# KRLabsOrg/verbatim-rag

Measured on AMD Instinct MI355X. Metric: query x chunk span-extractions/sec @512tok (ModernBERT-base extractor, chunks/s), higher is better.
Workload: dtype bf16

## Files before the change

### include/vrag_amd_debug.h

```cpp
#ifndef VRAG_AMD_DEBUG_H
#define VRAG_AMD_DEBUG_H

#include <stdint.h>

#ifdef __cplusplus
extern "C" {
#endif

int vrag_debug_gemm_ms(int32_t epi, int32_t M, int32_t N, int32_t K, int32_t iters, int32_t device, float* ms_out);
int vrag_debug_attn_ms(int32_t local, int32_t n_seqs, int32_t S, int32_t H, int32_t window, int32_t iters, int32_t device,
                       float* ms_out);
int vrag_debug_qkv_attn_ms(int32_t local, int32_t n_seqs, int32_t S, int32_t H, int32_t window, int32_t iters, int32_t flags,
                           int32_t device, float* ms_out);
typedef struct vrag_debug_attn_args {
  const uint16_t* q;
  const uint16_t* k;
  const uint16_t* vt;
  uint16_t* o;
  const int32_t* seq_row;
  const int32_t* seq_len;
  int32_t* blocks_out;
  int32_t rows, H, n_seqs;
  int32_t local, window, f16;
  int32_t blocks_cap;
  int32_t n_blocks;
  int32_t f16_saturated;
} vrag_debug_attn_args;
int vrag_debug_attn_run_ex(vrag_debug_attn_args* args, int32_t device);
int vrag_debug_attn_run(int32_t local, int32_t n_seqs, int32_t S, int32_t H, int32_t window, int32_t f16, const uint16_t* q,
                        const uint16_t* k, const uint16_t* vt, uint16_t* o, int32_t device);

typedef struct vrag_debug_gemm_args {
  const uint16_t* A;
  const uint16_t* W;
  const float* bias;
  const float* ln_s;
  const float* stats_in;
  const float* res_mu;
  const float* res_rstd;
  const float* res_g;
  const float* res_b;
  const float* rope_cos;
  const float* rope_sin;
  const int32_t* pos;
  const int32_t* tok_seq;
  const uint8_t* lo_in;
  float* out_f32;
  uint16_t* out_bf16;
  uint16_t* q;
  uint16_t* k;
  uint16_t* vt;
  float* ln_mu;
  float* ln_rstd;
  float* ln_shift;
  float* ln_shift_prev;
  uint16_t* resid_bf16;
  float* stats_part;
  uint8_t* lo_out;
  uint32_t* splade_rows;
  int32_t epi, M, N, K, f16, act_gelu;
  int32_t row0, rows;
  int32_t hidden, rope_rows, n_seqs;
  int32_t small_rows;
  float q_scale, fin_eps;
  int32_t config[7];
  int32_t f16_saturated;
} vrag_debug_gemm_args;
int vrag_debug_gemm_run(vrag_debug_gemm_args* args, int32_t device);

typedef struct vrag_debug_qkv_attn_args {
  const uint16_t* x;
  const uint16_t* w;
  const float* ln_s;
  const float* ln_mu;
  const float* ln_rstd;
  const float* rope_cos;
  const float* rope_sin;
  uint16_t* o;
  const int32_t* seq_row;
  const int32_t* seq_len;
  int32_t* groups_out;
  int32_t rows, H, nh, rope_rows, n_seqs;
  int32_t packer;
  int32_t local, window, f16;
  float q_scale;
  int32_t n_groups;
  int32_t f16_saturated;
} vrag_debug_qkv_attn_args;
int vrag_debug_qkv_attn_run(vrag_debug_qkv_attn_args* args, int32_t device);
int vrag_debug_pack_groups(const int32_t* seq_row, const int32_t* seq_len, int32_t n, int32_t packer, int32_t* out);

enum {
  VRAG_DEBUG_ROWS_EMBED_LN = 0,
  VRAG_DEBUG_ROWS_LAYERNORM = 1,
  VRAG_DEBUG_ROWS_RANGE_POOL = 2,
  VRAG_DEBUG_ROWS_LN_CLASSIFIER = 3,
  VRAG_DEBUG_ROWS_POOLER_CLASSIFIER = 4,
  VRAG_DEBUG_ROWS_SEQ_HEAD = 5
};
typedef struct vrag_debug_rows_args {
  float* h;
  const int32_t* ids;
  const float* E;
  const float* P;
  const int32_t* pos;
  const float* type_row;
  const int32_t* type_ids;
  const float* w;
  const float* bias;
  const int32_t* start;
  const int32_t* end;
  const int32_t* first_row;
  const int32_t* seq_row;
  const int32_t* seq_len;
  const float* Wp;
  const float* bp;
  const float* WdT;
  const float* bd;
  const float* wn;
  const float* bn;
  const float* Wc;
  const float* bc;
  float* out_f32;
  uint16_t* out16;
  uint16_t* out_lo;
  float* row_mean;
  float* pooled;
  int32_t op, H, rows;
  int32_t h_rows, out_rows;
  int32_t vocab, n_pos, n_types;
  int32_t num_labels;
  int32_t mode;
  int32_t gelu_first, split3;
  int32_t alias_f32;
  int32_t f16;
  int32_t no_sat;
  float eps;
  int32_t launch_status;
  int32_t f16_saturated;
} vrag_debug_rows_args;
int vrag_debug_rows_run(vrag_debug_rows_args* args, int32_t device);

enum {
  VRAG_DEBUG_GLUE_CVT_ROWS = 0,
  VRAG_DEBUG_GLUE_CVT_SPLIT3 = 1,
  VRAG_DEBUG_GLUE_LN_STATS_FINALIZE = 2,
  VRAG_DEBUG_GLUE_PACK_LAYOUT = 3,
  VRAG_DEBUG_GLUE_SPLADE_COMPACT = 4,
  VRAG_DEBUG_GLUE_PERMUTE_QKV_HEADS = 5
};
typedef struct vrag_debug_glue_args {
  const float* src;
  const float* col_scale;
  uint16_t* dst;
  uint16_t* dst_lo;
  float* row_sum;
  const float* part;
  float* mu;
  float* rstd;
  const float* shift_in;
  float* shift_out;
  float* shift_prev;
  const int32_t* packed;
  const int32_t* seq_row;
  const int32_t* seq_src;
  const int32_t* seq_len;
  int32_t* ids;
  int32_t* pos;
  int32_t* tok_seq;
  int32_t* counts;
// ... 166 lines not shown
```

### verbatim-rag_amd/_lib.py

```python
from __future__ import annotations

import ctypes as C
import os
import threading

_HERE = os.path.dirname(os.path.abspath(__file__))
_LOCK = threading.Lock()
_LIB = None

VRAG_OK = 0
ABI_VERSION = 6
PROF_CLASSES = (
    "embed", "layernorm", "gemm_qkv", "attn_global", "attn_local",
    "gemm_wo", "gemm_wi", "gemm_wo_mlp", "head", "qkv_attn_global", "qkv_attn_local",
)


class VragError(RuntimeError):

    def __init__(self, fn: str, status: int, message: str):
        super().__init__(f"{fn} failed (status {status}): {message}")
        self.status = status


# ... 135 lines not shown
                                      _LP, _LP, C.c_int64, _IP, _IP, _LP]),
    "vrag_split_sentences": (C.c_int, [C.c_void_p, _LP, C.c_int32, C.c_int32, _IP, _IP, _IP, C.c_int32]),
    "vrag_topk_fill_empty": (C.c_int, [C.c_void_p, C.c_void_p, C.c_int64, C.c_int32, C.c_void_p]),
    "vrag_sparse_index_create": (C.c_int, [C.c_int32, C.c_int64, _LP, _IP, _FP, C.c_int32, C.POINTER(_H)]),
    "vrag_sparse_index_destroy": (None, [_H]),
    "vrag_sparse_index_stats": (C.c_int, [_H, _LP, _LP, _LP]),
    "vrag_sparse_index_search": (C.c_int, [_H, _LP, _IP, _FP, C.c_int32, C.c_int32, _FP, _LP, C.c_void_p]),
    "vrag_sparse_index_search_filtered": (C.c_int, [_H, _LP, _IP, _FP, C.c_int32, C.c_int32, C.c_void_p, C.c_int64, _FP, _LP,
                                                    C.c_void_p]),
    "vrag_sparse_index_run_resident": (C.c_int, [_H, C.c_int32, C.c_int32, C.c_void_p]),
    "vrag_text_tokenize": (C.c_int, [C.c_void_p, _LP, C.c_int32, C.c_int32, C.c_int64, _IP, C.c_void_p, _LP]),
    "vrag_text_index_create": (C.c_int, [C.c_float, C.c_float, C.c_int32, C.POINTER(_H)]),
    "vrag_text_index_destroy": (None, [_H]),
    "vrag_text_index_add": (C.c_int, [_H, C.c_void_p, _LP, C.c_int32, C.c_int32]),
    "vrag_text_index_set_live": (C.c_int, [_H, C.c_void_p, C.c_int64]),
    "vrag_text_index_stats": (C.c_int, [_H, _LP, _LP, _LP, _LP, _LP]),
    "vrag_text_index_set_corpus_stats": (C.c_int, [_H, C.c_int64, C.c_int64]),
    "vrag_text_index_query_terms": (C.c_int, [_H, C.c_void_p, _LP, C.c_int32, C.c_int64, _LP, C.c_void_p, _IP, _LP, _LP]),
    "vrag_text_index_search": (C.c_int, [_H, _LP, C.c_void_p, _FP, C.c_int32, C.c_int32, C.c_void_p, C.c_int64, _FP, _LP]),
    "vrag_text_index_search_device": (C.c_int, [_H, _LP, C.c_void_p, _FP, C.c_int32, C.c_int32, C.c_void_p, C.c_int64, C.c_void_p,
                                                C.c_int64, C.c_int64, C.c_void_p, C.c_void_p, C.c_void_p]),
    "vrag_wordpiece_create": (C.c_int, [C.c_void_p, _LP, C.c_int32, C.c_int32, C.c_int32, C.c_int32, C.c_char_p, C.c_int32, C.c_int32,
                                        C.c_int32, C.POINTER(_H)]),
    "vrag_wordpiece_destroy": (None, [_H]),
    "vrag_wordpiece_encode": (C.c_int, [_H, C.c_void_p, _LP, C.c_int32, C.c_int32, C.c_int32, C.c_int64, _IP, _IP, C.c_void_p, _LP]),
    "vrag_bpe_create": (C.c_int, [C.c_int32, _IP, _IP, _IP, C.c_int32, _IP, _IP, C.c_void_p, _LP, _IP, C.c_int32, C.c_int32, C.c_int32,
                                  C.c_int32, C.c_int32, C.POINTER(_H)]),
    "vrag_bpe_destroy": (None, [_H]),
    "vrag_bpe_encode": (C.c_int, [_H, C.c_void_p, _LP, C.c_int32, C.c_int32, C.c_int32, C.c_int64, _IP, _IP, C.c_void_p, _LP]),
    "vrag_bpe_encode_offsets": (C.c_int, [_H, C.c_void_p, _LP, C.c_int32, C.c_int32, C.c_int32, C.c_int64, _IP, _IP, _IP, C.c_void_p, _LP]),
    "vrag_comm_get_unique_id": (C.c_int, [C.c_void_p]),
    "vrag_comm_create": (C.c_int, [C.c_void_p, C.c_int32, C.c_int32, C.c_int32, C.POINTER(_H)]),
    "vrag_comm_destroy": (None, [_H]),
    "vrag_comm_info": (C.c_int, [_H, _IP, _IP, _IP]),
    "vrag_comm_allgather": (C.c_int, [_H, C.c_void_p, C.c_void_p, C.c_int64, C.c_void_p]),
    "vrag_topk_allgather_merge": (C.c_int, [_H, C.c_void_p, C.c_void_p, C.c_int32, C.c_int32, C.c_int32, C.c_void_p, C.c_void_p,
                                            C.c_void_p]),
    "vrag_topk_merge": (C.c_int, [C.c_void_p, C.c_void_p, C.c_int32, C.c_int32, C.c_int32, C.c_int32, C.c_int64,
                                  C.c_int64, C.c_void_p, C.c_void_p, C.c_int32, C.c_int32, C.c_void_p]),
    "vrag_rrf_fuse": (C.c_int, [C.c_void_p, C.c_void_p, C.c_int32, C.c_int32, C.c_int32, C.c_void_p, C.c_void_p, C.c_int32,
                                C.c_int32, C.c_void_p]),
}


DEBUG_SIGNATURES = {
    "vrag_debug_gemm_ms": (C.c_int, [C.c_int32, C.c_int32, C.c_int32, C.c_int32, C.c_int32, C.c_int32, _FP]),
    "vrag_debug_attn_run": (C.c_int, [C.c_int32, C.c_int32, C.c_int32, C.c_int32, C.c_int32, C.c_int32, C.c_void_p, C.c_void_p,
                                      C.c_void_p, C.c_void_p, C.c_int32]),
    "vrag_debug_attn_run_ex": (C.c_int, [C.c_void_p, C.c_int32]),
    "vrag_debug_attn_ms": (C.c_int, [C.c_int32, C.c_int32, C.c_int32, C.c_int32, C.c_int32, C.c_int32, C.c_int32, _FP]),
    "vrag_debug_qkv_attn_ms": (C.c_int, [C.c_int32, C.c_int32, C.c_int32, C.c_int32, C.c_int32, C.c_int32, C.c_int32, C.c_int32, _FP]),
    "vrag_debug_gemm_run": (C.c_int, [C.c_void_p, C.c_int32]),
    "vrag_debug_qkv_attn_run": (C.c_int, [C.c_void_p, C.c_int32]),
    "vrag_debug_pack_groups": (C.c_int, [C.c_void_p, C.c_void_p, C.c_int32, C.c_int32, C.c_void_p]),
    "vrag_debug_rows_run": (C.c_int, [C.c_void_p, C.c_int32]),
    "vrag_debug_glue_run": (C.c_int, [C.c_void_p, C.c_int32]),
    "vrag_debug_topk_run": (C.c_int, [C.c_void_p, C.c_int32]),
    "vrag_debug_text_run": (C.c_int, [C.c_void_p, C.c_int32]),
    "vrag_debug_text_index_read": (C.c_int, [C.c_void_p, C.c_void_p]),
    "vrag_debug_token_spans": (C.c_int, [_FP, C.c_int64, _IP, _IP, _IP, _IP, C.c_int32, _LP, _IP, C.c_int32, C.c_float, C.c_int32, C.c_int32,
                                         C.c_int32, _IP, _IP, C.c_int32]),
    "vrag_debug_topk_launch_log_reset": (None, []),
    "vrag_debug_topk_launch_log_read": (C.c_int, [_IP, C.c_int32, _IP, _IP]),
}

DEBUG_TOPK_LAUNCH_IDS = {name: i for i, name in enumerate((
    "DENSE_BF16", "DENSE_F32", "MFMA", "MFMA2", "EXACT", "EXACT2", "SEED_THRESHOLD", "PF_PREFIX", "PF_COLLECT", "PF_COLLECT_MULTI",
    "PF_RESCORE_LIST", "PF_RESCORE", "PF_COMBINE", "SPARSE", "SPARSE_SCATTER", "SPARSE_MULTI", "MERGE_LISTS", "MERGE_SCAN"))}


class DebugGemmArgs(C.Structure):
    _fields_ = [(n, C.c_void_p) for n in (
        "A", "W", "bias", "ln_s", "stats_in", "res_mu", "res_rstd", "res_g", "res_b", "rope_cos", "rope_sin", "pos", "tok_seq",
        "lo_in", "out_f32", "out_bf16", "q", "k", "vt", "ln_mu", "ln_rstd", "ln_shift", "ln_shift_prev", "resid_bf16",
        "stats_part", "lo_out", "splade_rows")] + [(n, C.c_int32) for n in (
        "epi", "M", "N", "K", "f16", "act_gelu", "row0", "rows", "hidden", "rope_rows", "n_seqs", "small_rows")] + [
        ("q_scale", C.c_float), ("fin_eps", C.c_float), ("config", C.c_int32 * 7), ("f16_saturated", C.c_int32)]


class DebugQkvAttnArgs(C.Structure):
    _fields_ = [(n, C.c_void_p) for n in (
        "x", "w", "ln_s", "ln_mu", "ln_rstd", "rope_cos", "rope_sin", "o", "seq_row", "seq_len", "groups_out")] + [
        (n, C.c_int32) for n in ("rows", "H", "nh", "rope_rows", "n_seqs", "packer", "local", "window", "f16")] + [
        ("q_scale", C.c_float), ("n_groups", C.c_int32), ("f16_saturated", C.c_int32)]


class DebugAttnArgs(C.Structure):
    _fields_ = [(n, C.c_void_p) for n in ("q", "k", "vt", "o", "seq_row", "seq_len", "blocks_out")] + [
        (n, C.c_int32) for n in ("rows", "H", "n_seqs", "local", "window", "f16", "blocks_cap", "n_blocks", "f16_saturated")]


class DebugRowsArgs(C.Structure):
    _fields_ = [(n, C.c_void_p) for n in (
        "h", "ids", "E", "P", "pos", "type_row", "type_ids", "w", "bias", "start", "end", "first_row", "seq_row", "seq_len", "Wp",
        "bp", "WdT", "bd", "wn", "bn", "Wc", "bc", "out_f32", "out16", "out_lo", "row_mean", "pooled")] + [
        (n, C.c_int32) for n in ("op", "H", "rows", "h_rows", "out_rows", "vocab", "n_pos", "n_types", "num_labels", "mode",
                                 "gelu_first", "split3", "alias_f32", "f16", "no_sat")] + [
        ("eps", C.c_float), ("launch_status", C.c_int32), ("f16_saturated", C.c_int32)]


DEBUG_ROWS_OPS = {"embed_ln": 0, "layernorm": 1, "range_pool": 2, "ln_classifier": 3, "pooler_classifier": 4, "seq_head": 5}


class DebugGlueArgs(C.Structure):
    _fields_ = [(n, C.c_void_p) for n in (
        "src", "col_scale", "dst", "dst_lo", "row_sum", "part", "mu", "rstd", "shift_in", "shift_out", "shift_prev", "packed",
        "seq_row", "seq_src", "seq_len", "ids", "pos", "tok_seq", "counts", "idx", "val", "w", "s", "w_out", "s_out")] + [
        (n, C.c_int32) for n in ("op", "f16", "rows_dst", "rows_src", "cols", "interleave", "I", "out_rows", "rows", "ld", "row0",
                                 "H", "np", "nh", "alias_shift", "n_seqs", "n_packed", "pad_id", "V", "cap")] + [
        ("thr", C.c_float), ("eps", C.c_float), ("f16_saturated", C.c_int32)]


DEBUG_GLUE_OPS = {"cvt_rows": 0, "cvt_split3": 1, "ln_stats_finalize": 2, "pack_layout": 3, "splade_compact": 4,
                  "permute_qkv_heads": 5}



class DebugTopkArgs(C.Structure):
    _fields_ = [(n, C.c_void_p) for n in (
        "corpus", "w", "queries", "eps", "src", "w_out", "buf", "cnt", "thr_key", "thr_score", "out", "ovf", "done")] + [
        (n, C.c_int32) for n in ("op", "M", "N", "K", "corpus_rows", "nq", "nq_buf", "k", "cap", "pairs", "direct", "tile")] + [
        ("row_base", C.c_uint32)] + [
        (n, C.c_int32) for n in ("tile_stride", "tile_skip", "tile0", "n", "src_stride", "slices", "small_rows")] + [
        ("config", C.c_int32 * 7)]


DEBUG_TOPK_OPS = {"score_stage": 0, "queries": 1, "select": 2, "select_direct": 3, "rescue": 4, "merge": 5, "tau": 6}



class DebugTextArgs(C.Structure):
    _fields_ = [(n, C.c_void_p) for n in ("in", "out", "key", "row", "tf", "ukeys", "pstart", "prow", "ptf", "pkey")] + [
        (n, C.c_void_p * 4) for n in ("seg_keys", "seg_pstart", "seg_prow", "seg_ptf", "seg_df")] + [
        (n, C.c_void_p) for n in ("dl", "live", "allow", "acc", "kd", "qkeys", "tu", "df_out", "q_indptr", "w", "bound", "cand")] + [
        (n, C.c_int64 * 4) for n in ("seg_n_keys", "seg_n_post", "seg_row_lo", "seg_n_rows")] + [
        (n, C.c_int64) for n in ("n", "n_buf", "post_buf", "keys_buf", "n_rows", "rows_buf", "allow_rows", "n_terms", "terms_buf",
                                 "cand_buf", "corpus_n", "corpus_sum_dl", "n_post", "n_keys")] + [
        (n, C.c_int32) for n in ("op", "by_row", "row_bits", "unit", "n_segs", "nq", "kk")] + [
        ("k1", C.c_float), ("b", C.c_float), ("k1p1", C.c_float)]


DEBUG_TEXT_OPS = {"scan": 0, "sort": 1, "rle": 2, "fold": 3, "stats": 4, "lookup": 5, "score": 6}


class DebugTextIndexState(C.Structure):
    _fields_ = [(n, C.c_void_p * 2) for n in ("keys", "pstart", "prow", "ptf", "df")] + [
        (n, C.c_void_p) for n in ("dl", "kd", "live")] + [
        (n, C.c_int64 * 2) for n in ("row_lo", "seg_rows", "n_keys", "n_post")] + [
        (n, C.c_int64) for n in ("n_rows", "n_live", "sum_dl")] + [("n_segs", C.c_int32), ("with_data", C.c_int32)]


_DBG = None


def library_path() -> str:
    return os.environ.get("VRAG_AMD_LIB", os.path.join(_HERE, "libvrag_amd.so"))


def _preload_torch_hip_runtime() -> None:
    import importlib.util
    import sys

    if "torch" in sys.modules:
        return
    try:
        spec = importlib.util.find_spec("torch")
    except (ImportError, ValueError):
# ... 87 lines not shown
```

### verbatim-rag_amd/csrc/debug_api.hip

```cpp
#include "../../include/vrag_amd.h"
#include "../../include/vrag_amd_debug.h"

#include <algorithm>
#include <cstdlib>
#include <cstring>
#include <vector>

#include "attention.h"
#include "gemm_bf16.h"
#include "glue_kernels.h"
#include "host_util.h"
#include "norm_heads.h"
#include "qkv_attn.h"
#include "spans.h"
#include "topk_kernels.h"

using namespace vrag;

static inline int64_t align_up(int64_t v, int64_t a) { return (v + a - 1) / a * a; }

extern "C" {

int vrag_debug_gemm_ms(int32_t epi, int32_t M, int32_t N, int32_t K, int32_t iters, int32_t device, float* ms_out) {
  ARG_CHECK(ms_out && M > 0 && N % 128 == 0 && K % 64 == 0 && iters > 0, "bad arguments");
// ... 496 lines not shown
  g.A = (const bf16_t*)dev(iA, lo * K * 2);
  g.W = (const bf16_t*)dev(iW, 0);
  g.bias = (const float*)dev(ibias, 0);
  g.ln_s = (const float*)dev(ils, 0);
  g.stats_in = (const float*)dev(isin, lo * 8);
  g.stats_ld = (int)R;
  g.fin_eps = a->fin_eps;
  g.res_mu = (const float*)dev(irmu, lo * 4);
  g.res_rstd = (const float*)dev(irrs, lo * 4);
  g.res_g = (const float*)dev(irg, 0);
  g.res_b = (const float*)dev(irb, 0);
  g.rope_cos = (const float*)dev(icos, 0);
  g.rope_sin = (const float*)dev(isn, 0);
  g.pos = (const int*)dev(ipos, lo * 4);
  g.hidden = (int)H;
  g.vt_ld = (int)R;
  g.q_scale = a->q_scale;
  g.tok_seq = (const int*)dev(itok, lo * 4);
  g.splade_rows = (unsigned*)dev(ispl, 0);
  g.lo_in = (const unsigned char*)dev(ilo_in, lo * N);
  g.lo_out = (unsigned char*)dev(ilo_out, lo * N);
  g.out_f32 = (float*)dev(iof, lo * N * 4);
  g.out_bf16 = (bf16_t*)dev(iob, lo * NO * 2);
  g.q = (bf16_t*)dev(iq, lo * H * 2);
  g.k = (bf16_t*)dev(ik, lo * H * 2);
  g.vt = (bf16_t*)dev(ivt, lo * 2);
  g.ln_mu = (const float*)dev(imu, lo * 4);
  g.ln_rstd = (const float*)dev(irs, lo * 4);
  g.ln_shift = (const float*)dev(ish, lo * 4);
  g.ln_shift_prev = (float*)dev(ishp, lo * 4);
  g.resid_bf16 = (bf16_t*)dev(ires, lo * N * 2);
  g.stats_part = (float*)dev(isp, lo * 8);
  const int thr = gemm_small_m_threshold(-1);
  if (e == hipSuccess) e = hipDeviceSynchronize();
  if (e == hipSuccess) {
    if (a->small_rows >= 0) gemm_small_m_threshold(a->small_rows);
    e = launch_gemm((GemmEpi)epi, g, 0);
    const GemmConfig c = gemm_last_config();
    gemm_small_m_threshold(thr);
    const int32_t cfg[7] = {c.bm, c.bn, c.wm, c.wn, c.ns, c.hw, c.kch};
    std::memcpy(a->config, cfg, sizeof(cfg));
  }
  if (e == hipSuccess) e = hipDeviceSynchronize();
  unsigned saturated = 0;
  if (e == hipSuccess) e = hipMemcpy(&saturated, sat.p, 4, hipMemcpyDeviceToHost);
  if (e == hipSuccess) a->f16_saturated = saturated ? 1 : 0;
  std::vector<unsigned char> canary(kCanary);
  const char* clobbered = nullptr;
  for (Buf& b : bufs) {
    if (e != hipSuccess) break;
    e = hipMemcpy(canary.data(), b.dev.as<char>() + b.bytes, kCanary, hipMemcpyDeviceToHost);
    if (e == hipSuccess && !clobbered && std::any_of(canary.begin(), canary.end(), [](unsigned char v) { return v != kCanaryByte; }))
      clobbered = b.name;
    if (e == hipSuccess && b.host_out) e = hipMemcpy(b.host_out, b.dev.p, b.bytes, hipMemcpyDeviceToHost);
  }
  if (e != hipSuccess) {
    set_error("debug gemm run failed: %s", hipGetErrorString(e));
    return VRAG_ERR_HIP;
  }
  if (clobbered) {
    set_error("debug gemm run: the launch wrote past the end of %s", clobbered);
    return VRAG_ERR_HIP;
  }
  return VRAG_OK;
}

int vrag_debug_pack_groups(const int32_t* seq_row, const int32_t* seq_len, int32_t n, int32_t packer, int32_t* out) {
  ARG_CHECK(seq_row && seq_len && out && n > 0 && (packer == 0 || packer == 1), "bad arguments");
  for (int s = 0; s < n; ++s) ARG_CHECK(seq_len[s] >= 1 && seq_len[s] <= kFusedMaxSeq, "seq_len[%d] = %d outside 1..%d", s, seq_len[s], kFusedMaxSeq);
  static_assert(sizeof(int4) == 4 * sizeof(int32_t), "descriptor layout");
  int4* g = reinterpret_cast<int4*>(out);
  return packer ? pack_groups_best_fit(seq_row, seq_len, 0, n, g) : fused_pack_groups(seq_row, seq_len, 0, n, g);
}

int vrag_debug_qkv_attn_run(vrag_debug_qkv_attn_args* a, int32_t device) {
  ARG_CHECK(a, "null arguments");
  ARG_CHECK(a->x && a->w && a->rope_cos && a->rope_sin && a->o && a->seq_row && a->seq_len && a->groups_out, "null required pointer");
  ARG_CHECK(!(a->ln_mu || a->ln_rstd) || (a->ln_mu && a->ln_rstd && a->ln_s), "the fold needs ln_mu, ln_rstd and ln_s");
  ARG_CHECK(a->nh > 0 && a->H == 64 * a->nh, "H (%d) must be 64 * nh (%d)", a->H, a->nh);
  ARG_CHECK(a->rows > 0 && a->rows % kRowPad == 0, "rows (%d) must be a positive multiple of %d", a->rows, kRowPad);
  ARG_CHECK((int64_t)a->rows * a->H < ((int64_t)1 << 31), "rows * H must stay below 2^31");
  ARG_CHECK(a->rope_rows > 0 && a->n_seqs > 0 && (a->packer == 0 || a->packer == 1), "bad rope_rows / n_seqs / packer");
  ARG_CHECK(!a->local || a->window >= 0, "bad window");
  ARG_CHECK(device >= 0, "bad device %d", device);
  const int n = a->n_seqs;
  for (int s = 0; s < n; ++s) {
    const int row = a->seq_row[s], len = a->seq_len[s];
    ARG_CHECK(len >= 1 && len <= kFusedMaxSeq, "seq_len[%d] = %d outside 1..%d", s, len, kFusedMaxSeq);
    ARG_CHECK(row >= 0 && row % kSeqAlign == 0, "seq_row[%d] = %d must be a non-negative multiple of %d", s, row, kSeqAlign);
    ARG_CHECK((int64_t)row + 64 * ((len + 63) / 64) <= a->rows, "sequence %d (row %d, %d tokens): its last wave reads past row %d", s, row, len, a->rows);
  }
  {
    std::vector<int> order(n);
    for (int s = 0; s < n; ++s) order[s] = s;
    std::sort(order.begin(), order.end(), [&](int l, int r) { return a->seq_row[l] < a->seq_row[r]; });
    for (int i = 0; i + 1 < n; ++i)
      ARG_CHECK(a->seq_row[order[i]] + a->seq_len[order[i]] <= a->seq_row[order[i + 1]], "sequences %d and %d overlap", order[i], order[i + 1]);
  }
  if (vrag_device_count() <= device) {
    set_error("no HIP device %d visible", device);
    return VRAG_ERR_NO_DEVICE;
  }
  HIP_TRY(hipSetDevice(device));
  const size_t R = (size_t)a->rows, H = (size_t)a->H;
  const bool fold = a->ln_mu != nullptr;
  std::vector<int4> groups((size_t)n * 8);
  const int n_groups = a->packer ? pack_groups_best_fit(a->seq_row, a->seq_len, 0, n, groups.data())
                                 : fused_pack_groups(a->seq_row, a->seq_len, 0, n, groups.data());
  std::memcpy(a->groups_out, groups.data(), (size_t)n_groups * 8 * sizeof(int4));
  a->n_groups = n_groups;

  constexpr size_t kCanary = 4096;
  constexpr unsigned char kCanaryByte = 0xA5;
  DevBuf x, w, wh, ls, lsh, mu, rstd, cs, sn, o, d_groups, sat;
  hipError_t e = x.alloc(R * H * 2);
  if (e == hipSuccess) e = w.alloc(3 * H * H * 2);
  if (e == hipSuccess) e = wh.alloc(3 * H * H * 2);
  if (e == hipSuccess) e = cs.alloc((size_t)a->rope_rows * 32 * 4);
  if (e == hipSuccess) e = sn.alloc((size_t)a->rope_rows * 32 * 4);
  if (e == hipSuccess) e = o.alloc(R * H * 2 + kCanary);
  if (e == hipSuccess) e = d_groups.alloc((size_t)n_groups * 8 * sizeof(int4));
  if (e == hipSuccess) e = sat.alloc(4);
  if (e == hipSuccess) e = hipMemset(sat.p, 0, 4);
  if (e == hipSuccess) e = hipMemcpy(x.p, a->x, R * H * 2, hipMemcpyHostToDevice);
  if (e == hipSuccess) e = hipMemcpy(w.p, a->w, 3 * H * H * 2, hipMemcpyHostToDevice);
  if (e == hipSuccess) e = hipMemcpy(cs.p, a->rope_cos, (size_t)a->rope_rows * 32 * 4, hipMemcpyHostToDevice);
  if (e == hipSuccess) e = hipMemcpy(sn.p, a->rope_sin, (size_t)a->rope_rows * 32 * 4, hipMemcpyHostToDevice);
  if (e == hipSuccess) e = hipMemcpy(o.p, a->o, R * H * 2, hipMemcpyHostToDevice);
  if (e == hipSuccess) e = hipMemset(o.as<char>() + R * H * 2, kCanaryByte, kCanary);
  if (e == hipSuccess) e = hipMemcpy(d_groups.p, groups.data(), (size_t)n_groups * 8 * sizeof(int4), hipMemcpyHostToDevice);
  if (fold) {
    if (e == hipSuccess) e = ls.alloc(3 * H * 4);
    if (e == hipSuccess) e = lsh.alloc((3 * H + 64) * 4);
    if (e == hipSuccess) e = mu.alloc(R * 4);
    if (e == hipSuccess) e = rstd.alloc(R * 4);
    if (e == hipSuccess) e = hipMemset(lsh.p, 0, (3 * H + 64) * 4);
    if (e == hipSuccess) e = hipMemcpy(ls.p, a->ln_s, 3 * H * 4, hipMemcpyHostToDevice);
    if (e == hipSuccess) e = hipMemcpy(mu.p, a->ln_mu, R * 4, hipMemcpyHostToDevice);
    if (e == hipSuccess) e = hipMemcpy(rstd.p, a->ln_rstd, R * 4, hipMemcpyHostToDevice);
  }
  if (e == hipSuccess) e = permute_qkv_heads(w.as<bf16_t>(), fold ? ls.as<float>() : nullptr, (int)H, a->nh, wh.as<bf16_t>(),
                                             fold ? lsh.as<float>() : nullptr, nullptr);
  if (e == hipSuccess) e = hipDeviceSynchronize();
  if (e == hipSuccess) {
    QkvAttnParams f{};
    f.x = x.as<bf16_t>();
    f.w = wh.as<bf16_t>();
    f.ln_mu = fold ? mu.as<float>() : nullptr;
    f.ln_rstd = fold ? rstd.as<float>() : nullptr;
    f.ln_s = fold ? lsh.as<float>() : nullptr;
    f.rope_cos = cs.as<float>();
    f.rope_sin = sn.as<float>();
    f.rope_rows = a->rope_rows;
    f.o = o.as<bf16_t>();
    f.groups = d_groups.as<int4>();
    f.n_groups = n_groups;
    f.H = (int)H;
    f.nh = a->nh;
    f.Tp = (int)R;
    f.window = a->window;
    f.op_dtype = a->f16 ? kOpF16 : kOpBf16;
    f.q_scale = a->q_scale;
    f.debug_flags = 0;
    f.f16_sat = sat.as<unsigned>();
    e = launch_qkv_attention(f, a->local != 0, 0);
  }
  if (e == hipSuccess) e = hipDeviceSynchronize();
  unsigned saturated = 0;
  if (e == hipSuccess) e = hipMemcpy(&saturated, sat.p, 4, hipMemcpyDeviceToHost);
  std::vector<unsigned char> canary(kCanary);
  if (e == hipSuccess) e = hipMemcpy(canary.data(), o.as<char>() + R * H * 2, kCanary, hipMemcpyDeviceToHost);
  if (e == hipSuccess) e = hipMemcpy(a->o, o.p, R * H * 2, hipMemcpyDeviceToHost);
  if (e != hipSuccess) {
    set_error("debug fused attention run failed: %s", hipGetErrorString(e));
    return VRAG_ERR_HIP;
  }
  if (std::any_of(canary.begin(), canary.end(), [](unsigned char v) { return v != kCanaryByte; })) {
    set_error("debug fused attention run: the launch wrote past the end of o");
    return VRAG_ERR_HIP;
  }
  a->f16_saturated = saturated ? 1 : 0;
  return VRAG_OK;
}

int vrag_debug_rows_run(vrag_debug_rows_args* a, int32_t device) {
  ARG_CHECK(a, "null arguments");
  const int op = a->op, H = a->H, rows = a->rows;
  ARG_CHECK(op >= VRAG_DEBUG_ROWS_EMBED_LN && op <= VRAG_DEBUG_ROWS_SEQ_HEAD, "op %d is not a row launcher", op);
  ARG_CHECK(H >= 1 && H <= 65536, "H (%d) outside 1..65536: the buffers cannot be sized", H);
  ARG_CHECK(rows >= 0, "rows (%d) is negative: the buffers cannot be sized", rows);
  ARG_CHECK(a->out_rows >= rows, "out_rows (%d) below rows (%d)", a->out_rows, rows);
  ARG_CHECK(device >= 0, "bad device %d", device);
  const bool embed = op == VRAG_DEBUG_ROWS_EMBED_LN, ln = op == VRAG_DEBUG_ROWS_LAYERNORM, range = op == VRAG_DEBUG_ROWS_RANGE_POOL;
  const bool lncls = op == VRAG_DEBUG_ROWS_LN_CLASSIFIER, pooler = op == VRAG_DEBUG_ROWS_POOLER_CLASSIFIER;
  const bool seqh = op == VRAG_DEBUG_ROWS_SEQ_HEAD;
  const bool classifier = lncls || pooler || seqh || (range && a->mode == 0);
  if (embed) {
    ARG_CHECK(a->ids && a->E && a->w && a->out_f32 && a->out16, "embed_ln needs ids, E, w, out_f32 and out16");
    ARG_CHECK(a->vocab >= 1, "vocab (%d) must be positive", a->vocab);
    for (int r = 0; r < rows; ++r) ARG_CHECK(a->ids[r] >= 0 && a->ids[r] < a->vocab, "ids[%d] = %d outside the %d rows of E", r, a->ids[r], a->vocab);
    if (a->P && a->pos) {
      ARG_CHECK(a->n_pos >= 1, "n_pos (%d) must be positive", a->n_pos);
      for (int r = 0; r < rows; ++r) ARG_CHECK(a->pos[r] >= 0 && a->pos[r] < a->n_pos, "pos[%d] = %d outside the %d rows of P", r, a->pos[r], a->n_pos);
    }
    if (a->P && a->type_row) {
      ARG_CHECK(a->n_types >= 1, "n_types (%d) must be positive", a->n_types);
      if (a->type_ids)
        for (int r = 0; r < rows; ++r)
          ARG_CHECK(a->type_ids[r] >= 0 && a->type_ids[r] < a->n_types, "type_ids[%d] = %d outside the %d rows of type_row", r, a->type_ids[r], a->n_types);
    }
  } else {
    ARG_CHECK(a->h, "h is required");
    ARG_CHECK(a->h_rows >= 1, "h_rows (%d) must be positive", a->h_rows);
  }
  if (ln || lncls) ARG_CHECK(a->h_rows >= rows, "h holds %d rows, the launch reads %d", a->h_rows, rows);
  if (ln) ARG_CHECK(!(a->alias_f32 && a->out_f32), "alias_f32 makes h the fp32 output: out_f32 must be null");
  if (range) {
    ARG_CHECK(a->start && a->end && a->out_f32, "range_pool needs start, end and out_f32");
    for (int r = 0; r < rows; ++r) {
      ARG_CHECK(a->start[r] >= 0, "start[%d] = %d is negative", r, a->start[r]);
      ARG_CHECK(a->end[r] < a->h_rows, "end[%d] = %d is past the last row %d of h (end is inclusive)", r, a->end[r], a->h_rows - 1);
      ARG_CHECK(a->start[r] <= a->end[r], "range %d is empty (start %d > end %d): the kernel would divide by zero", r, a->start[r], a->end[r]);
    }
  }
  if (lncls) ARG_CHECK(a->w && a->out_f32, "ln_classifier needs w and out_f32");
  if (pooler) {
    ARG_CHECK(a->first_row && a->Wp && a->bp && a->out_f32, "pooler_classifier needs first_row, Wp, bp and out_f32");
    for (int r = 0; r < rows; ++r)
      ARG_CHECK(a->first_row[r] >= 0 && a->first_row[r] < a->h_rows, "first_row[%d] = %d outside the %d rows of h", r, a->first_row[r], a->h_rows);
  }
  if (seqh) {
    ARG_CHECK(a->seq_row && a->seq_len && a->pooled && a->WdT && a->wn && a->out_f32, "seq_head needs seq_row, seq_len, pooled, WdT, wn and out_f32");
    for (int r = 0; r < rows; ++r) {
      ARG_CHECK(a->seq_len[r] >= 1, "seq_len[%d] = %d must be at least 1", r, a->seq_len[r]);
      ARG_CHECK(a->seq_row[r] >= 0, "seq_row[%d] = %d is negative", r, a->seq_row[r]);
      ARG_CHECK((int64_t)a->seq_row[r] + a->seq_len[r] <= a->h_rows, "sequence %d (row %d, %d tokens) ends past the %d rows of h", r, a->seq_row[r], a->seq_len[r], a->h_rows);
    }
  }
  if (classifier) {
    ARG_CHECK(a->num_labels >= 1, "num_labels (%d) must be at least 1 where a classifier runs", a->num_labels);
    ARG_CHECK(a->Wc && a->bc, "the classifier needs Wc and bc");
  }
  if (vrag_device_count() <= device) {
    set_error("no HIP device %d visible", device);
    return VRAG_ERR_NO_DEVICE;
  }
// ... 558 lines not shown
```

### verbatim-rag_amd/csrc/qkv_attn.hip

```cpp
#include "host_util.h"
#include "qkv_attn.h"

#include <algorithm>
#include <cstdlib>
#include <type_traits>
#include <vector>

#ifdef VRAG_DEBUG_API
#define VRAG_DBG(bit) ((p.debug_flags & (bit)) != 0)
#else
#define VRAG_DBG(bit) false
#endif

namespace vrag {

constexpr int QA_WB = 192 * 128;
constexpr int QA_XOFF = 2 * QA_WB;
constexpr int QA_TAB = 131072;
constexpr int QA_MU = QA_TAB, QA_RS = QA_TAB + 2048, QA_LS = QA_TAB + 4096;
constexpr int QA_CA = QA_TAB + 5120, QA_SA = QA_CA + 4096, QA_CB = QA_SA + 4096, QA_SB = QA_CB + 2048;
constexpr int QA_SMEM = QA_SB + 2048;
constexpr int QA_V_OFF = 65536;

constexpr float QA_LAZY = 8.0f;
// ... 197 lines not shown
    for (int kq = 0; kq < 2; ++kq)
#pragma unroll
      for (int hf = 0; hf < 2; ++hf) {
        lsum[kq][np][hf] = f32x4{0.f, 0.f, 0.f, 0.f};
        if constexpr (FOLD) lsum[kq][np][hf] = *reinterpret_cast<const f32x4*>(l_ls + (kq == 0 ? 64 : 0) + 32 * hf + dd);
      }
  }
  auto rope_rows = [&](int a0, int rt, const f32x4 (&ls)[2][2], const f32x2 (&cs)[2][2], const f32x2 (&sns)[2][2], float mu, float rs, float scale,
                       V8 (&out)[2]) {
    const bool live = qrow0 + rt * 16 + l15 < S;
#pragma unroll
    for (int np = 0; np < 2; ++np) {
      const f32x4& l1 = ls[np][0];
      const f32x4& l2 = ls[np][1];
#pragma unroll
      for (int h = 0; h < 2; ++h) {
        const int j0 = 2 * h;
        f32x2 x1 = {acc[a0 + np][rt][j0], acc[a0 + np][rt][j0 + 1]}, x2 = {acc[a0 + 2 + np][rt][j0], acc[a0 + 2 + np][rt][j0 + 1]};
        if constexpr (FOLD) {
          x1 = pk_fma(splat2(-mu), f32x2{l1[j0], l1[j0 + 1]}, x1) * rs;
          x2 = pk_fma(splat2(-mu), f32x2{l2[j0], l2[j0 + 1]}, x2) * rs;
        }
        const f32x2 c = cs[np][h], sn = sns[np][h];
        const f32x2 o1 = pk_fma(-x2, sn, x1 * c) * scale, o2 = pk_fma(x1, sn, x2 * c) * scale;
#pragma unroll
        for (int e = 0; e < 2; ++e) {
          if constexpr (!std::is_same<T, bf16_t>::value) {
            out[0][np * 4 + j0 + e] = live ? Op<T>::to(o1[e], p.f16_sat) : (T)0.f;
            out[1][np * 4 + j0 + e] = live ? Op<T>::to(o2[e], p.f16_sat) : (T)0.f;
          } else {
            out[0][np * 4 + j0 + e] = Op<T>::to(o1[e], p.f16_sat);
            out[1][np * 4 + j0 + e] = Op<T>::to(o2[e], p.f16_sat);
          }
        }
      }
    }
  };
  V8 qf[4][2];
#pragma unroll
  for (int rt = 0; rt < 4; ++rt) {
    const float mu = FOLD ? l_mu[rt * 16 + l15] : 0.f, rs = FOLD ? l_rs[rt * 16 + l15] : 1.f;
    f32x2 c[2][2], sn[2][2];
#pragma unroll
    for (int np = 0; np < 2; ++np) {
      const int dd = np * 16 + 4 * g;
      const f32x4 ca = *reinterpret_cast<const f32x4*>(smem + QA_CA + (((qrow0 >> 4) + rt) * 32 + dd) * 4);
      const f32x4 sa = *reinterpret_cast<const f32x4*>(smem + QA_SA + (((qrow0 >> 4) + rt) * 32 + dd) * 4);
#pragma unroll
      for (int h = 0; h < 2; ++h) {
        const int j0 = 2 * h;
        const f32x2 ca2 = {ca[j0], ca[j0 + 1]}, sa2 = {sa[j0], sa[j0 + 1]}, cb2 = {cb[np][j0], cb[np][j0 + 1]}, sb2 = {sb[np][j0], sb[np][j0 + 1]};
        c[np][h] = pk_fma(-sa2, sb2, ca2 * cb2);
        sn[np][h] = pk_fma(ca2, sb2, sa2 * cb2);
      }
    }
    V8 kf[2];
    rope_rows(4, rt, lsum[0], c, sn, mu, rs, 1.0f, kf);
    const int row = srow0 + rt * 16 + l15;
#pragma unroll
    for (int s = 0; s < 2; ++s) *reinterpret_cast<V8*>(smem + row * 128 + (((4 * s + g) ^ ((row >> 1) & 7)) << 4)) = kf[s];
    rope_rows(0, rt, lsum[1], c, sn, mu, rs, p.q_scale, qf[rt]);
  }
  __syncthreads();

  f32x4 ot[4][4];
  f32x4 lo[4];
#pragma unroll
  for (int c = 0; c < 4; ++c) {
    lo[c] = f32x4{0.f, 0.f, 0.f, 0.f};
#pragma unroll
    for (int dt = 0; dt < 4; ++dt) ot[c][dt] = f32x4{0.f, 0.f, 0.f, 0.f};
  }
  float m_run[4] = {0.f, 0.f, 0.f, 0.f};
  bool seen[4] = {false, false, false, false};
  V8 ones;
#pragma unroll
  for (int j = 0; j < 8; ++j) ones[j] = (T)1.0f;
  const int W = p.window;
  int kt_lo = 0, kt_hi = (S - 1) >> 6;
  if constexpr (LOCAL) {
    kt_lo = max(0, qrow0 - W) >> 6;
    kt_hi = min(S - 1, qrow0 + 63 + W) >> 6;
  }
  const int ksw = (l15 >> 1) & 7;
  if (active && !VRAG_DBG(1)) {
    for (int kt = kt_lo; kt <= kt_hi; ++kt) {
      bool cut[2][2];
#pragma unroll
      for (int u = 0; u < 2; ++u) {
        const int q_lo = qrow0 + 32 * u;
#pragma unroll
        for (int t2 = 0; t2 < 2; ++t2) {
          const int kh = kt * 64 + t2 * 32;
          bool outside = kh >= S || q_lo >= S;
          cut[u][t2] = kh + 31 >= S;
          if constexpr (LOCAL) {
            outside = outside || (kh + 31 < q_lo - W) || (kh > q_lo + 31 + W);
            cut[u][t2] = cut[u][t2] || (kh < q_lo + 31 - W) || (kh + 31 > q_lo + W);
          }
          cut[u][t2] = cut[u][t2] || outside;
        }
      }
      V8 pf[4][2];
      {
        f32x4 st[4][4];
#pragma unroll
        for (int c = 0; c < 4; ++c) {
          const float seed = -m_run[c];
#pragma unroll
          for (int kb = 0; kb < 4; ++kb) st[c][kb] = f32x4{seed, seed, seed, seed};
        }
#pragma unroll
        for (int kb = 0; kb < 4; ++kb) {
          const char* krow = smem + ((kbase + kt) * 64 + kb * 16 + l15) * 128;
          const V8 k0 = *reinterpret_cast<const V8*>(krow + ((g ^ ksw) << 4));
          const V8 k1 = *reinterpret_cast<const V8*>(krow + (((4 + g) ^ ksw) << 4));
#pragma unroll
          for (int c = 0; c < 4; ++c) {
            st[c][kb] = Op<T>::mfma16(k0, qf[c][0], st[c][kb]);
            st[c][kb] = Op<T>::mfma16(k1, qf[c][1], st[c][kb]);
          }
        }
        float mx[4];
#pragma unroll
        for (int c = 0; c < 4; ++c) {
          const int u = c >> 1;
          mx[c] = -INFINITY;
#pragma unroll
          for (int t2 = 0; t2 < 2; ++t2) {
            if (cut[u][t2]) {
              const int qi = qrow0 + 16 * c + l15;
              int lo_k = 0, hi_k = S - 1;
              if constexpr (LOCAL) {
                lo_k = max(0, qi - W);
                hi_k = min(S - 1, qi + W);
              }
              const unsigned span = hi_k >= lo_k ? (unsigned)(hi_k - lo_k) : 0u;
              int d0 = hi_k >= lo_k ? kt * 64 + t2 * 32 + 4 * g - lo_k : -100000;
              asm volatile("" : "+v"(d0));
#pragma unroll
              for (int h2 = 0; h2 < 2; ++h2)
#pragma unroll
                for (int r = 0; r < 4; ++r) {
                  const bool ok = (unsigned)(d0 + 16 * h2 + r) <= span;
                  st[c][2 * t2 + h2][r] = ok ? st[c][2 * t2 + h2][r] : -INFINITY;
                }
            }
            const f32x4& a = st[c][2 * t2];
            const f32x4& b2 = st[c][2 * t2 + 1];
            mx[c] = max3f(mx[c], max3f(a[0], a[1], a[2]), max3f(a[3], b2[0], b2[1]));
            mx[c] = max3f(mx[c], b2[2], b2[3]);
          }
        }
        bool move = false;
#pragma unroll
        for (int c = 0; c < 4; ++c) {
          const bool qlive = qrow0 + 16 * c + l15 < S;
          move = move || (qlive && (mx[c] > QA_LAZY || (!seen[c] && mx[c] > -INFINITY)));
        }
        if (__any(move)) {
#pragma unroll
          for (int c = 0; c < 4; ++c) {
            float m_all = fmaxf(mx[c], __shfl_xor(mx[c], 16, 64));
            m_all = fmaxf(m_all, __shfl_xor(m_all, 32, 64));
            const bool has = m_all > -INFINITY;
            const float delta = seen[c] ? fmaxf(m_all, 0.f) : (has ? m_all : 0.f);
            const float alpha = seen[c] ? __builtin_amdgcn_exp2f(-delta) : 1.0f;
            seen[c] = seen[c] || has;
            m_run[c] += delta;
#pragma unroll
            for (int kb = 0; kb < 4; ++kb)
#pragma unroll
              for (int r = 0; r < 4; ++r) st[c][kb][r] -= delta;
#pragma unroll
            for (int dt = 0; dt < 4; ++dt)
#pragma unroll
              for (int r = 0; r < 4; ++r) ot[c][dt][r] *= alpha;
#pragma unroll
            for (int r = 0; r < 4; ++r) lo[c][r] *= alpha;
          }
        }
#pragma unroll
        for (int c = 0; c < 4; ++c)
#pragma unroll
          for (int t2 = 0; t2 < 2; ++t2)
#pragma unroll
            for (int j = 0; j < 8; ++j) pf[c][t2][j] = (T)__builtin_amdgcn_exp2f(st[c][2 * t2 + (j >> 2)][j & 3]);
      }
#pragma unroll
      for (int t2 = 0; t2 < 2; ++t2) {
#pragma unroll
        for (int c = 0; c < 4; ++c) lo[c] = Op<T>::mfma16(ones, pf[c][t2], lo[c]);
#pragma unroll
        for (int dt = 0; dt < 4; ++dt) {
          const V8 vf = *reinterpret_cast<const V8*>(smem + QA_V_OFF + (dt * 16 + l15) * 1024 + ((((kbase + kt) * 8 + t2 * 4 + g) ^ l15) << 4));
#pragma unroll
          for (int c = 0; c < 4; ++c) ot[c][dt] = Op<T>::mfma16(vf, pf[c][t2], ot[c][dt]);
        }
      }
    }
  }
  __syncthreads();

  if (active) {
    char* stg = smem + wave * 8192;
#pragma unroll
    for (int rt = 0; rt < 4; ++rt) {
      const int row = rt * 16 + l15;
      const bool live = qrow0 + row < S;
      const float inv = live ? 1.0f / lo[rt][0] : 0.f;
#pragma unroll
      for (int db = 0; db < 4; ++db) {
        V4 o;
#pragma unroll
        for (int j = 0; j < 4; ++j) o[j] = live ? Op<T>::to(ot[rt][db][j] * inv, p.f16_sat) : (T)0.f;
        const int c16 = db * 2 + (g >> 1);
        *reinterpret_cast<V4*>(stg + row * 128 + ((c16 ^ (row & 7)) << 4) + ((g & 1) << 3)) = o;
      }
    }
#pragma unroll
    for (int it = 0; it < 8; ++it) {
      const int row = it * 8 + (lane >> 3), c16 = lane & 7;
      const f32x4 v = *reinterpret_cast<const f32x4*>(stg + row * 128 + ((c16 ^ (row & 7)) << 4));
      if (qrow0 + row < S && !VRAG_DBG(8)) store16_nt(reinterpret_cast<T*>(p.o) + (size_t)(wrow0 + row) * H + head * 64 + c16 * 8, v);
    }
  }
}

template <bool LOCAL, bool FOLD, typename T>
static hipError_t launch_t(const QkvAttnParams& p, hipStream_t stream) {
  const hipError_t e = set_max_dynamic_lds<&qkv_attn_kernel<LOCAL, FOLD, T>>(QA_SMEM);
  if (e != hipSuccess) return e;
  const int grid = ((p.n_groups + 7) / 8) * 8 * p.nh;
  hipLaunchKernelGGL((qkv_attn_kernel<LOCAL, FOLD, T>), dim3(grid), dim3(512), QA_SMEM, stream, p);
  return hipGetLastError();
}

hipError_t launch_qkv_attention(const QkvAttnParams& p, bool local, hipStream_t stream) {
  if (p.op_dtype == kOpF16 && !p.f16_sat) return hipErrorInvalidValue;
  if (p.n_groups <= 0) return hipSuccess;
  if (p.H % 64 != 0 || p.H != p.nh * 64 || (size_t)p.Tp * p.H >= (size_t)1 << 31) return hipErrorInvalidValue;
  const bool fold = p.ln_mu != nullptr;
  if (p.op_dtype == kOpF16) {
    if (fold) return local ? launch_t<true, true, f16_t>(p, stream) : launch_t<false, true, f16_t>(p, stream);
    return local ? launch_t<true, false, f16_t>(p, stream) : launch_t<false, false, f16_t>(p, stream);
  }
  if (fold) return local ? launch_t<true, true, bf16_t>(p, stream) : launch_t<false, true, bf16_t>(p, stream);
  return local ? launch_t<true, false, bf16_t>(p, stream) : launch_t<false, false, bf16_t>(p, stream);
}

__global__ void permute_qkv_heads_kernel(const bf16_t* __restrict__ w, const float* __restrict__ s, int H, int nh,
                                         bf16_t* __restrict__ w_out, float* __restrict__ s_out) {
  const int orow = blockIdx.x;
  const int head = orow / 192, part = (orow % 192) / 64, d = orow % 64;
  const int src = part * H + head * 64 + d;
  for (int i = threadIdx.x; i < H; i += blockDim.x) w_out[(size_t)orow * H + i] = w[(size_t)src * H + i];
  if (threadIdx.x == 0 && s && s_out) s_out[orow] = s[src];
}

hipError_t permute_qkv_heads(const bf16_t* w, const float* s, int H, int nh, bf16_t* w_out, float* s_out, hipStream_t stream) {
  hipLaunchKernelGGL(permute_qkv_heads_kernel, dim3(3 * H), dim3(256), 0, stream, w, s, H, nh, w_out, s_out);
  return hipGetLastError();
}

int fused_pack_groups(const int* seq_row, const int* seq_len, int seq0, int seq1, int4* out) {
  int n = 0, used = 8;
  for (int s = seq0; s < seq1; ++s) {
    const int need = (seq_len[s] + 63) / 64;
    if (used + need > 8) {
      for (int w = 0; w < 8; ++w) out[n * 8 + w] = int4{0, 0, 0, 0};
      ++n;
      used = 0;
    }
    for (int j = 0; j < need; ++j) out[(n - 1) * 8 + used + j] = int4{seq_row[s] + 64 * j, seq_len[s], used, 0};
    used += need;
  }
  return n;
}

int pack_groups_best_fit(const int* seq_row, const int* seq_len, int seq0, int seq1, int4* out) {
  std::vector<int> by_need[9];
  for (int s = seq0; s < seq1; ++s) by_need[std::min(8, (seq_len[s] + 63) / 64)].push_back(s);
// ... 26 lines not shown
```

Before: 7795.

## Specialize local-attention window tiles to skip masked MFMA blocks

```diff
diff --git a/include/vrag_amd_debug.h b/include/vrag_amd_debug.h
--- a/include/vrag_amd_debug.h
+++ b/include/vrag_amd_debug.h
@@ -86,6 +86,7 @@
   float q_scale;
   int32_t n_groups;
   int32_t f16_saturated;
+  int32_t debug_flags;
 } vrag_debug_qkv_attn_args;
 int vrag_debug_qkv_attn_run(vrag_debug_qkv_attn_args* args, int32_t device);
 int vrag_debug_pack_groups(const int32_t* seq_row, const int32_t* seq_len, int32_t n, int32_t packer, int32_t* out);
diff --git a/verbatim-rag_amd/_lib.py b/verbatim-rag_amd/_lib.py
--- a/verbatim-rag_amd/_lib.py
+++ b/verbatim-rag_amd/_lib.py
@@ -241,7 +241,7 @@
     _fields_ = [(n, C.c_void_p) for n in (
         "x", "w", "ln_s", "ln_mu", "ln_rstd", "rope_cos", "rope_sin", "o", "seq_row", "seq_len", "groups_out")] + [
         (n, C.c_int32) for n in ("rows", "H", "nh", "rope_rows", "n_seqs", "packer", "local", "window", "f16")] + [
-        ("q_scale", C.c_float), ("n_groups", C.c_int32), ("f16_saturated", C.c_int32)]
+        ("q_scale", C.c_float), ("n_groups", C.c_int32), ("f16_saturated", C.c_int32), ("debug_flags", C.c_int32)]
 
 
 class DebugAttnArgs(C.Structure):
diff --git a/verbatim-rag_amd/csrc/debug_api.hip b/verbatim-rag_amd/csrc/debug_api.hip
--- a/verbatim-rag_amd/csrc/debug_api.hip
+++ b/verbatim-rag_amd/csrc/debug_api.hip
@@ -602,6 +602,7 @@
   ARG_CHECK((int64_t)a->rows * a->H < ((int64_t)1 << 31), "rows * H must stay below 2^31");
   ARG_CHECK(a->rope_rows > 0 && a->n_seqs > 0 && (a->packer == 0 || a->packer == 1), "bad rope_rows / n_seqs / packer");
   ARG_CHECK(!a->local || a->window >= 0, "bad window");
+  ARG_CHECK(a->debug_flags == 0 || a->debug_flags == 32, "debug_flags (%d) must be 0 or 32", a->debug_flags);
   ARG_CHECK(device >= 0, "bad device %d", device);
   const int n = a->n_seqs;
   for (int s = 0; s < n; ++s) {
@@ -681,7 +682,7 @@
     f.window = a->window;
     f.op_dtype = a->f16 ? kOpF16 : kOpBf16;
     f.q_scale = a->q_scale;
-    f.debug_flags = 0;
+    f.debug_flags = a->debug_flags;
     f.f16_sat = sat.as<unsigned>();
     e = launch_qkv_attention(f, a->local != 0, 0);
   }
diff --git a/verbatim-rag_amd/csrc/qkv_attn.hip b/verbatim-rag_amd/csrc/qkv_attn.hip
--- a/verbatim-rag_amd/csrc/qkv_attn.hip
+++ b/verbatim-rag_amd/csrc/qkv_attn.hip
@@ -303,10 +303,25 @@
     kt_lo = max(0, qrow0 - W) >> 6;
     kt_hi = min(S - 1, qrow0 + 63 + W) >> 6;
   }
-  const int ksw = (l15 >> 1) & 7;
-  if (active && !VRAG_DBG(1)) {
-    for (int kt = kt_lo; kt <= kt_hi; ++kt) {
-      bool cut[2][2];
+  constexpr int QA_GENERIC = 0, QA_FIRST = 1, QA_MID = 2, QA_LAST = 3;
+  bool diag_first[4], diag_last[4];
+#pragma unroll
+  for (int r = 0; r < 4; ++r) {
+    diag_first[r] = 4 * g + r >= l15;
+    diag_last[r] = 4 * g + r <= l15;
+  }
+  auto tile = [&](auto mode_c, const int kt) {
+    constexpr int MODE = decltype(mode_c)::value;
+    const int ln = [&] {
+      int v = lane;
+      if constexpr (LOCAL) asm volatile("" : "+v"(v));
+      return v;
+    }();
+    const int g = ln >> 4, l15 = ln & 15, ksw = (l15 >> 1) & 7;
+    auto blk = [](int c, int kb) { return MODE == QA_FIRST ? kb >= c : MODE == QA_LAST ? kb <= c : true; };
+    auto step = [&](int c, int t2) { return blk(c, 2 * t2) || blk(c, 2 * t2 + 1); };
+    bool cut[2][2];
+    if constexpr (MODE == QA_GENERIC) {
 #pragma unroll
       for (int u = 0; u < 2; ++u) {
         const int q_lo = qrow0 + 32 * u;
@@ -322,33 +337,37 @@
           cut[u][t2] = cut[u][t2] || outside;
         }
       }
-      V8 pf[4][2];
-      {
-        f32x4 st[4][4];
-#pragma unroll
-        for (int c = 0; c < 4; ++c) {
-          const float seed = -m_run[c];
-#pragma unroll
-          for (int kb = 0; kb < 4; ++kb) st[c][kb] = f32x4{seed, seed, seed, seed};
-        }
-#pragma unroll
-        for (int kb = 0; kb < 4; ++kb) {
-          const char* krow = smem + ((kbase + kt) * 64 + kb * 16 + l15) * 128;
-          const V8 k0 = *reinterpret_cast<const V8*>(krow + ((g ^ ksw) << 4));
-          const V8 k1 = *reinterpret_cast<const V8*>(krow + (((4 + g) ^ ksw) << 4));
-#pragma unroll
-          for (int c = 0; c < 4; ++c) {
+    }
+    V8 pf[4][2];
+    {
+      f32x4 st[4][4];
+#pragma unroll
+      for (int c = 0; c < 4; ++c) {
+        const float seed = -m_run[c];
+#pragma unroll
+        for (int kb = 0; kb < 4; ++kb)
+          if (blk(c, kb)) st[c][kb] = f32x4{seed, seed, seed, seed};
+      }
+#pragma unroll
+      for (int kb = 0; kb < 4; ++kb) {
+        const char* krow = smem + ((kbase + kt) * 64 + kb * 16 + l15) * 128;
+        const V8 k0 = *reinterpret_cast<const V8*>(krow + ((g ^ ksw) << 4));
+        const V8 k1 = *reinterpret_cast<const V8*>(krow + (((4 + g) ^ ksw) << 4));
+#pragma unroll
+        for (int c = 0; c < 4; ++c)
+          if (blk(c, kb)) {
             st[c][kb] = Op<T>::mfma16(k0, qf[c][0], st[c][kb]);
             st[c][kb] = Op<T>::mfma16(k1, qf[c][1], st[c][kb]);
           }
-        }
-        float mx[4];
-#pragma unroll
-        for (int c = 0; c < 4; ++c) {
-          const int u = c >> 1;
-          mx[c] = -INFINITY;
-#pragma unroll
-          for (int t2 = 0; t2 < 2; ++t2) {
+      }
+      float mx[4];
+#pragma unroll
+      for (int c = 0; c < 4; ++c) {
+        const int u = c >> 1;
+        mx[c] = -INFINITY;
+#pragma unroll
+        for (int t2 = 0; t2 < 2; ++t2) {
+          if constexpr (MODE == QA_GENERIC) {
             if (cut[u][t2]) {
               const int qi = qrow0 + 16 * c + l15;
               int lo_k = 0, hi_k = S - 1;
@@ -367,58 +386,97 @@
                   st[c][2 * t2 + h2][r] = ok ? st[c][2 * t2 + h2][r] : -INFINITY;
                 }
             }
-            const f32x4& a = st[c][2 * t2];
-            const f32x4& b2 = st[c][2 * t2 + 1];
+          } else if constexpr (MODE != QA_MID) {
+            if (c >> 1 == t2) {
+#pragma unroll
+              for (int r = 0; r < 4; ++r) st[c][c][r] = (MODE == QA_FIRST ? diag_first[r] : diag_last[r]) ? st[c][c][r] : -INFINITY;
+            }
+          }
+          const f32x4& a = st[c][2 * t2];
+          const f32x4& b2 = st[c][2 * t2 + 1];
+          if (blk(c, 2 * t2) && blk(c, 2 * t2 + 1)) {
             mx[c] = max3f(mx[c], max3f(a[0], a[1], a[2]), max3f(a[3], b2[0], b2[1]));
             mx[c] = max3f(mx[c], b2[2], b2[3]);
-          }
-        }
-        bool move = false;
+          } else if (blk(c, 2 * t2)) {
+            mx[c] = max3f(mx[c], max3f(a[0], a[1], a[2]), a[3]);
+          } else if (blk(c, 2 * t2 + 1)) {
+            mx[c] = max3f(mx[c], max3f(b2[0], b2[1], b2[2]), b2[3]);
+          }
+        }
+      }
+      bool move = false;
+#pragma unroll
+      for (int c = 0; c < 4; ++c) {
+        const bool qlive = qrow0 + 16 * c + l15 < S;
+        move = move || (qlive && (mx[c] > QA_LAZY || (!seen[c] && mx[c] > -INFINITY)));
+      }
+      if (__any(move)) {
 #pragma unroll
         for (int c = 0; c < 4; ++c) {
-          const bool qlive = qrow0 + 16 * c + l15 < S;
-          move = move || (qlive && (mx[c] > QA_LAZY || (!seen[c] && mx[c] > -INFINITY)));
-        }
-        if (__any(move)) {
-#pragma unroll
-          for (int c = 0; c < 4; ++c) {
-            float m_all = fmaxf(mx[c], __shfl_xor(mx[c], 16, 64));
-            m_all = fmaxf(m_all, __shfl_xor(m_all, 32, 64));
-            const bool has = m_all > -INFINITY;
-            const float delta = seen[c] ? fmaxf(m_all, 0.f) : (has ? m_all : 0.f);
-            const float alpha = seen[c] ? __builtin_amdgcn_exp2f(-delta) : 1.0f;
-            seen[c] = seen[c] || has;
-            m_run[c] += delta;
-#pragma unroll
-            for (int kb = 0; kb < 4; ++kb)
+          float m_all = fmaxf(mx[c], __shfl_xor(mx[c], 16, 64));
+          m_all = fmaxf(m_all, __shfl_xor(m_all, 32, 64));
+          const bool has = m_all > -INFINITY;
+          const float delta = seen[c] ? fmaxf(m_all, 0.f) : (has ? m_all : 0.f);
+          const float alpha = seen[c] ? __builtin_amdgcn_exp2f(-delta) : 1.0f;
+          seen[c] = seen[c] || has;
+          m_run[c] += delta;
+#pragma unroll
+          for (int kb = 0; kb < 4; ++kb)
+            if (blk(c, kb)) {
 #pragma unroll
               for (int r = 0; r < 4; ++r) st[c][kb][r] -= delta;
-#pragma unroll
-            for (int dt = 0; dt < 4; ++dt)
-#pragma unroll
-              for (int r = 0; r < 4; ++r) ot[c][dt][r] *= alpha;
-#pragma unroll
-            for (int r = 0; r < 4; ++r) lo[c][r] *= alpha;
-          }
-        }
+            }
+#pragma unroll
+          for (int dt = 0; dt < 4; ++dt)
+#pragma unroll
+            for (int r = 0; r < 4; ++r) ot[c][dt][r] *= alpha;
+#pragma unroll
+          for (int r = 0; r < 4; ++r) lo[c][r] *= alpha;
+        }
+      }
+#pragma unroll
+      for (int c = 0; c < 4; ++c)
+#pragma unroll
+        for (int t2 = 0; t2 < 2; ++t2)
+          if (step(c, t2)) {
+#pragma unroll
+            for (int j = 0; j < 8; ++j)
+              pf[c][t2][j] = blk(c, 2 * t2 + (j >> 2)) ? (T)__builtin_amdgcn_exp2f(st[c][2 * t2 + (j >> 2)][j & 3]) : (T)0.f;
+          }
+    }
+#pragma unroll
+    for (int t2 = 0; t2 < 2; ++t2) {
+#pragma unroll
+      for (int c = 0; c < 4; ++c)
+        if (step(c, t2)) lo[c] = Op<T>::mfma16(ones, pf[c][t2], lo[c]);
+#pragma unroll
+      for (int dt = 0; dt < 4; ++dt) {
+        const V8 vf = *reinterpret_cast<const V8*>(smem + QA_V_OFF + (dt * 16 + l15) * 1024 + ((((kbase + kt) * 8 + t2 * 4 + g) ^ l15) << 4));
 #pragma unroll
         for (int c = 0; c < 4; ++c)
-#pragma unroll
-          for (int t2 = 0; t2 < 2; ++t2)
-#pragma unroll
-            for (int j = 0; j < 8; ++j) pf[c][t2][j] = (T)__builtin_amdgcn_exp2f(st[c][2 * t2 + (j >> 2)][j & 3]);
-      }
-#pragma unroll
-      for (int t2 = 0; t2 < 2; ++t2) {
-#pragma unroll
-        for (int c = 0; c < 4; ++c) lo[c] = Op<T>::mfma16(ones, pf[c][t2], lo[c]);
-#pragma unroll
-        for (int dt = 0; dt < 4; ++dt) {
-          const V8 vf = *reinterpret_cast<const V8*>(smem + QA_V_OFF + (dt * 16 + l15) * 1024 + ((((kbase + kt) * 8 + t2 * 4 + g) ^ l15) << 4));
-#pragma unroll
-          for (int c = 0; c < 4; ++c) ot[c][dt] = Op<T>::mfma16(vf, pf[c][t2], ot[c][dt]);
-        }
-      }
+          if (step(c, t2)) ot[c][dt] = Op<T>::mfma16(vf, pf[c][t2], ot[c][dt]);
+      }
+    }
+  };
+  if (active && !VRAG_DBG(1)) {
+    if constexpr (LOCAL) {
+      const bool fixed = W == 64 && !VRAG_DBG(32);
+      const int own = qrow0 >> 6;
+      if (fixed && qrow0 >= 64 && qrow0 + 127 < S) {
+        tile(std::integral_constant<int, QA_FIRST>{}, own - 1);
+        tile(std::integral_constant<int, QA_MID>{}, own);
+        tile(std::integral_constant<int, QA_LAST>{}, own + 1);
+      } else if (fixed && qrow0 == 0 && 127 < S) {
+        tile(std::integral_constant<int, QA_MID>{}, own);
+        tile(std::integral_constant<int, QA_LAST>{}, own + 1);
+      } else if (fixed && qrow0 >= 64 && qrow0 + 64 == S) {
+        tile(std::integral_constant<int, QA_FIRST>{}, own - 1);
+        tile(std::integral_constant<int, QA_MID>{}, own);
+      } else {
+        for (int kt = kt_lo; kt <= kt_hi; ++kt) tile(std::integral_constant<int, QA_GENERIC>{}, kt);
+      }
+    } else {
+      for (int kt = kt_lo; kt <= kt_hi; ++kt) tile(std::integral_constant<int, QA_GENERIC>{}, kt);
     }
   }
   __syncthreads();
```

Result: faster. 7899, median of 6 (+1.3%).
